# MAGPIE-ICL/synthPy

Measured on AMD Instinct MI355X. Metric: ray-steps/sec (+ rays/sec to detector), 1e7 rays x 512^3 volume, higher is better.
Workload: dtype f64

## Files before the change

include/synthray.h:

```cpp
#ifndef SYNTHRAY_H
#define SYNTHRAY_H

#include <stddef.h>
#include <stdint.h>

#ifdef __cplusplus
extern "C" {
#endif

#define SR_OK 0
#define SR_ERR_INVALID (-1)
#define SR_ERR_HIP (-2)
#define SR_ERR_RCCL (-3)
#define SR_ERR_STATE (-4)

typedef struct sr_volume sr_volume;
typedef struct sr_rays sr_rays;
typedef struct sr_image sr_image;
typedef struct sr_comm sr_comm;

int sr_init(int device);
int sr_device_count(void);
int sr_synchronize(void);
int sr_device_memory(int64_t *free_bytes, int64_t *total_bytes);
// ... 85 lines not shown
} sr_trace_stats;

int sr_trace(const sr_volume *v, const double *s0, int64_t n_rays, const sr_trace_params *p,
             double *sf, double *rf, double *Jf, sr_trace_stats *stats);

int sr_ray_to_jones(const double *sf, int64_t n_rays, double extent, int probing_axis, int row_order,
                    double *rf, double *Jf);

int sr_rays_create(sr_rays **out, int64_t n_rays);
int sr_rays_upload(sr_rays *r, const double *s0);
int sr_rays_upload_part(sr_rays *r, const double *s0, int64_t n, int64_t first, int last);
int sr_rays_generate(sr_rays *r, int beam_type, double size_a, double size_b, double divergence, double ne_extent,
                     int probing_axis, uint64_t seed, uint64_t first_ray);
int sr_rays_trace(sr_rays *r, const sr_volume *v, const sr_trace_params *p, sr_trace_stats *stats);
int sr_rays_trace_stats(sr_rays *r, sr_trace_stats *stats);

int sr_rays_tile_segments(const sr_rays *r);
int sr_rays_tile_records(const sr_rays *r);
double sr_tile_min_density(void);
int sr_rays_download(const sr_rays *r, double *sf, double *rf, double *Jf);
int sr_rays_download_s0(const sr_rays *r, double *s0);
int sr_rays_error_bound(const sr_rays *r, float *bound);
int64_t sr_rays_count(const sr_rays *r);
int sr_rays_handoff_download(const sr_rays *r, double *rec);
int sr_rays_set_bbox(sr_rays *r, const double *bbox);
int sr_rays_get_bbox(const sr_rays *r, double *bbox, int *known);
int sr_rays_handoff_upload(sr_rays *r, const double *rec);
int sr_rays_handoff_send(sr_rays *r, sr_comm *comm, int peer);
int sr_rays_handoff_recv(sr_rays *r, sr_comm *comm, int peer);
void sr_rays_destroy(sr_rays *r);

enum {
  SR_OP_DIST = 0,
  SR_OP_LENS = 1,
  SR_OP_CIRC_AP = 2,
  SR_OP_CIRC_STOP = 3,
  SR_OP_RECT_AP = 4,
  SR_OP_KNIFE = 5,
  SR_OP_SCALE = 6,
  SR_OP_PHASE = 7
};
typedef struct {
  int32_t op;
  int32_t iarg;
  double a;
  double b;
// ... 72 lines not shown
```

synthpy_amd/_ffi.py:

```python
from __future__ import annotations

import ctypes as C
import os

import numpy as np

_HERE = os.path.dirname(os.path.abspath(__file__))
LIB_PATH = os.environ.get("SYNTHRAY_LIB") or os.path.join(_HERE, "libsynthray.so")


class SynthrayError(RuntimeError):
    """A libsynthray call returned a negative status."""


class Optic(C.Structure):
    _fields_ = [("op", C.c_int32), ("iarg", C.c_int32), ("a", C.c_double), ("b", C.c_double)]


class TraceParams(C.Structure):
    _fields_ = [("t_end", C.c_double), ("extent", C.c_double), ("dt", C.c_double), ("probing_axis", C.c_int32),
                ("row_order", C.c_int32), ("substeps", C.c_int32), ("sort_rays", C.c_int32), ("precision", C.c_int32),
                ("handoff", C.c_int32)]


# ... 57 lines not shown
    "sr_volume_sample_aux": (_i, [_vp, _vp, _i64, _vp]),
    "sr_volume_project": (_i, [_vp, _vp, C.POINTER(C.c_uint32)]),
    "sr_volume_omega": (_d, [_vp]),
    "sr_volume_bytes": (_i64, [_vp]),
    "sr_volume_destroy": (None, [_vp]),
    "sr_trace": (_i, [_vp, _vp, _i64, C.POINTER(TraceParams), _vp, _vp, _vp, C.POINTER(TraceStats)]),
    "sr_ray_to_jones": (_i, [_vp, _i64, _d, _i, _i, _vp, _vp]),
    "sr_rays_create": (_i, [_pp, _i64]),
    "sr_rays_download_s0": (_i, [_vp, _vp]),
    "sr_rays_error_bound": (_i, [_vp, _vp]),
    "sr_rays_generate": (_i, [_vp, _i, _d, _d, _d, _d, _i, C.c_uint64, C.c_uint64]),
    "sr_rays_upload": (_i, [_vp, _vp]),
    "sr_rays_upload_part": (_i, [_vp, _vp, _i64, _i64, _i]),
    "sr_rays_trace": (_i, [_vp, _vp, C.POINTER(TraceParams), C.POINTER(TraceStats)]),
    "sr_release_caches": (_i, []),
    "sr_rays_trace_stats": (_i, [_vp, C.POINTER(TraceStats)]),
    "sr_rays_tile_segments": (_i, [_vp]),
    "sr_tile_min_density": (_d, []),
    "sr_rays_tile_records": (_i, [_vp]),
    "sr_rays_set_bbox": (_i, [_vp, _vp]),
    "sr_rays_get_bbox": (_i, [_vp, _vp, C.POINTER(C.c_int)]),
    "sr_rays_download": (_i, [_vp, _vp, _vp, _vp]),
    "sr_rays_count": (_i64, [_vp]),
    "sr_rays_destroy": (None, [_vp]),
    "sr_optics": (_i, [C.POINTER(Optic), _i, _d, _i64, _vp, _vp, _vp, _vp]),
    "sr_hist2d": (_i, [_vp, _vp, _i64, _i, _i, _d, _d, _d, _d, _vp]),
    "sr_interferogram": (_i, [_vp, _vp, _vp, _i64, _i, _i, _d, _d, _d, _d, _vp, _vp]),
    "sr_interfere_ref_beam": (_i, [_vp, _vp, _i64, _d, _d, _vp]),
    "sr_image_create": (_i, [_pp, _i, _i, _i, _d, _d, _d, _d]),
    "sr_image_zero": (_i, [_vp]),
    "sr_image_download": (_i, [_vp, _vp]),
    "sr_image_amplitude": (_i, [_vp, _vp]),
    "sr_image_counts_f64": (_i, [_vp, _vp]),
    "sr_rays_optics": (_i, [_vp, C.POINTER(Optic), _i, C.POINTER(DepositParams), _vp, _vp]),
    "sr_image_bytes": (_i64, [_vp]),
    "sr_image_destroy": (None, [_vp]),
    "sr_rays_deposit": (_i, [_vp, C.POINTER(Optic), _i, C.POINTER(DepositParams), _vp, C.POINTER(DepositStats)]),
    "sr_rays_refine": (_i, [_vp, _i, _vp, _vp, _vp, C.POINTER(C.c_int64)]),
    "sr_image_create_intensity": (_i, [_pp, _i, _i, _i, _d, _d, _d, _d]),
    "sr_rays_deposit_intensity": (_i, [_vp, C.POINTER(Optic), _i, _vp, _i, _i, _vp, C.POINTER(DepositStats)]),
    "sr_intensity2d": (_i, [_vp, _vp, _vp, _i64, _vp, _i, _i, _i, _d, _d, _d, _d, _vp]),
    "sr_image_rotation": (_i, [_vp, _i, _i, _d, _vp]),
    "sr_comm_unique_id": (_i, [_vp]),
    "sr_comm_create": (_i, [_pp, _vp, _i, _i]),
    "sr_image_reduce": (_i, [_vp, _vp, _i]),
    "sr_comm_ranks": (_i, [_vp, C.POINTER(C.c_int), C.POINTER(C.c_int)]),
# ... 45 lines not shown
```

synthpy_amd/csrc/common.hpp:

```cpp
#pragma once
#include <hip/hip_runtime.h>

#include <cstdarg>
#include <cstdint>
#include <cstdio>
#include <map>
#include <string>
#include <type_traits>
#include <vector>

#include "synthray.h"

namespace sr {

constexpr double kC = 299792458.0;

void set_error(const char *fmt, ...);
int fail(int code, const char *fmt, ...);

#define SR_HIP(call)                                                                         \
  do {                                                                                       \
    hipError_t e_ = (call);                                                                  \
    if (e_ != hipSuccess)                                                                    \
      return sr::fail(SR_ERR_HIP, "%s failed: %s (%s:%d)", #call, hipGetErrorString(e_),     \
// ... 99 lines not shown
  mutable std::map<int, void *> step_tabs;
};

struct sr_rays {
  int64_t n = 0;
  int64_t cap = 0;
  double bbox[6] = {0, 0, 0, 0, 0, 0};
  bool have_bbox = false;
  bool bbox_given = false;
  double *s0 = nullptr;
  double *sf = nullptr;
  double *rf = nullptr;
  double *Jf = nullptr;
  uint32_t *perm = nullptr;
  uint32_t *keys = nullptr;
  uint32_t *bins = nullptr;
  uint32_t *sort_tmp = nullptr;
  int64_t bins_cap = 0;
  uint32_t *fb_list = nullptr;
  unsigned long long *counters = nullptr;
  double *rec = nullptr;
  double *rec2 = nullptr;
  uint32_t *order2 = nullptr;
  double *strag_rec = nullptr;
  unsigned long long *strag_snap = nullptr;
  int strag_snap_cap = 0;
  bool have_s0 = false, traced = false, sorted = false, have_rec = false;
  bool counters_carry = false;
  int tile_segs = 0;
  int tile_segs_run = 0;
  bool tile_rec = false;
  float *guard = nullptr;
  const sr_volume *last_vol = nullptr;
  sr_trace_params last_p{};
  void *guard_set = nullptr;
  std::vector<char> guard_set_host;
  bool guard_live = false;
  double guard_len = 0;
};

namespace sr {
int retrace_f64(const sr_rays *r, const uint32_t *list, const unsigned long long *count);
int download_rows(const sr_rays *r, double *sf, double *rf, double *Jf, int64_t ld, int64_t off, double *staging);
}

struct sr_image {
// ... 8 lines not shown
```

synthpy_amd/csrc/trace.hip:

```cpp
#include <algorithm>
#include <cmath>
#include <cstdlib>
#include <cstring>

#include "common.hpp"

namespace {

struct VolDev {
  const float4 *P;
  const float *L;
  const double *g[3];
  const double *rg[3];
  int na, nb, nc;
  double omega;
  const double *K;
  const double *Q;
  double verdet;
  int64_t OS;
  const double *R;
};

constexpr int64_t kSC = 8;
__device__ __forceinline__ int64_t col8(const VolDev &V, int ib, int ic) { return ((int64_t)ib * V.nc + ic) * 8; }
// ... 236 lines not shown
    run += v[q];
  }
  const int lane = threadIdx.x & 63, wid = threadIdx.x >> 6;
  uint32_t incl = run;
  for (int off = 1; off < 64; off <<= 1) {
    const uint32_t up = __shfl_up(incl, off, 64);
    if (lane >= off) incl += up;
  }
  if (lane == 63) wsum[wid] = incl;
  __syncthreads();
  uint32_t woff = 0;
  for (int w = 0; w < wid; ++w) woff += wsum[w];
  uint32_t ex = woff + incl - run;
#pragma unroll
  for (int q = 0; q < 8; ++q) {
    if (base + q < n) bins[base + q] = ex;
    ex += v[q];
  }
  if (threadIdx.x == 255) sums[blockIdx.x] = woff + incl;
}
__global__ void k_scan_add(uint32_t *__restrict__ bins, int64_t n, const uint32_t *__restrict__ sums) {
  const int64_t i = blockIdx.x * (int64_t)blockDim.x + threadIdx.x;
  if (i < n) bins[i] += sums[i / kScanPerBlock];
}

__device__ __forceinline__ void project(int a, int row_order, double extent, int64_t N, int64_t j, double pa, double pb,
                                        double pc, double va, double vb, double vc, double amp, double phase, double pol,
                                        double *__restrict__ rf, double *__restrict__ Jf) {
  const double tb = (pa - extent) / va;
  double q0 = pb - vb * tb, q2 = pc - vc * tb;
  double a1 = atan(vb / va), a3 = atan(vc / va);
  if (a == 1 && row_order == SR_ROWS_LEGACY) {
    double t = q0;
    q0 = q2;
    q2 = t;
    t = a1;
    a1 = a3;
    a3 = t;
  }
  rf[j] = q0;
  rf[N + j] = a1;
  rf[2 * N + j] = q2;
  rf[3 * N + j] = a3;
  if (Jf) {
    double sp, cp, so, co;
    sincos(phase, &sp, &cp);
// ... 385 lines not shown
    sr::dev_free(r->bins);
    r->bins = nullptr;
    r->bins_cap = 0;
    int rc = sr::dev_alloc(&r->bins, (size_t)(ncount + nsb));
    if (rc) return rc;
    r->bins_cap = ncount + nsb;
  }
  if (!r->sort_tmp) {
    int rc = sr::dev_alloc(&r->sort_tmp, (size_t)2 * (size_t)std::max(r->cap, N));
    if (rc) return rc;
  }
  uint32_t *sums = r->bins + ncount, *tkeys = r->sort_tmp, *trays = r->sort_tmp + N;
  hipLaunchKernelGGL(k_bin_count, dim3(n_wg), dim3(256), 0, st, (const uint32_t *)r->keys, N, lo_bits, n_coarse, r->bins, n_wg);
  hipLaunchKernelGGL(k_scan_blocks, dim3((unsigned)nsb), dim3(256), 0, st, r->bins, ncount, sums);
  hipLaunchKernelGGL(k_scan, dim3(1), dim3(1024), 0, st, sums, nsb);
  hipLaunchKernelGGL(k_scan_add, dim3(sr::grid_for(ncount, 256)), dim3(256), 0, st, r->bins, ncount, (const uint32_t *)sums);
  hipLaunchKernelGGL(k_bin_coarse, dim3(n_wg), dim3(256), 0, st, (const uint32_t *)r->keys, N, lo_bits, n_coarse,
                     (const uint32_t *)r->bins, n_wg, tkeys, trays);
  hipLaunchKernelGGL(k_bin_fine, dim3((unsigned)n_coarse), dim3(1024), 0, st, (const uint32_t *)tkeys, (const uint32_t *)trays, N,
                     lo_bits, n_coarse, (const uint32_t *)r->bins, n_wg, out);
  return SR_OK;
}

int bin_by_band(sr_rays *r, const sr_volume *v, const TileGeom &g, const double *rec, uint32_t *out, hipStream_t st) {
  const int64_t N = r->n;
  const int64_t n_bands = (v->nb - 1 + g.band - 1) / g.band;
  const int64_t n_keys = n_bands * (int64_t)(v->nc - 1) * g.band;
  int bits = 1;
  while (((int64_t)1 << bits) < n_keys) ++bits;
  const int shift = std::max(0, bits - 22);
  const int64_t key_max = ((n_keys - 1) >> shift) + 1;
  bits = 1;
  while (((int64_t)1 << bits) <= key_max) ++bits;
  const int lo_bits = std::min(11, (bits + 1) / 2);
  const int n_coarse = (int)(key_max >> lo_bits) + 1;
  SR_CHECK(n_coarse <= kBinMaxDigits + 1, "band key of %lld does not fit the LDS counters of the ray binning", (long long)key_max);
  const unsigned nblk = sr::grid_for(N, 256);
  if (rec)
    hipLaunchKernelGGL(k_keys_band_rec, dim3(nblk), dim3(256), 0, st, vol_dev(v), rec, N, g.band, (uint32_t)key_max, shift, r->keys);
  else
    hipLaunchKernelGGL(k_keys_band, dim3(nblk), dim3(256), 0, st, vol_dev(v), (const double *)r->s0, N, v->axis, g.band, (uint32_t)key_max,
                       shift, r->keys);
  return bin_rays(r, N, lo_bits, n_coarse, out, st);
}

constexpr double kTileMinDensity = 8.0;
struct TilePlan {
  TileGeom g;
  int seg;
  bool rec;
};

struct TraceKnobs {
  int f64_tile = -1;
  bool tile_records = true;
  bool strag_beside = true;
  bool aux_one_pass = false;
  TileGeom tile{};
  int tile_seg = 0;
  std::vector<double> cuts;
};
TraceKnobs trace_knobs() {
  TraceKnobs k;
  if (const char *e = getenv("SYNTHRAY_F64_TILE")) k.f64_tile = e[0] == '0' ? 0 : (e[0] == '1' ? 1 : -1);
  if (const char *e = getenv("SYNTHRAY_TILE_RECORDS")) k.tile_records = e[0] != '0';
  if (const char *e = getenv("SYNTHRAY_STRAGGLERS")) k.strag_beside = e[0] != 's';
  if (const char *e = getenv("SYNTHRAY_AUX_ONE_PASS")) k.aux_one_pass = e[0] == '1';
  if (const char *e = getenv("SYNTHRAY_TILE")) {
    int a, b, c, d, f;
    if (sscanf(e, "%d,%d,%d,%d,%d", &a, &b, &c, &d, &f) == 5 && a >= 2 && b >= 2 && c >= 0 && d >= 1 && f >= 1 && a * b <= SR_TILE_THREADS) {
      k.tile = TileGeom{a, b, c, d};
      k.tile_seg = f;
    }
  }
  if (const char *e = getenv("SYNTHRAY_TILE_CUTS"))
    for (const char *q = e; *q;) {
      char *end = nullptr;
      const double x = strtod(q, &end);
      if (end == q) break;
      k.cuts.push_back(x);
      q = *end == ',' ? end + 1 : end;
    }
  return k;
}
double beam_cells(const sr_rays *r, const sr_volume *v) {
  const double all = (double)(v->nb - 1) * (double)(v->nc - 1);
  if (!r || !r->have_bbox) return all;
  double cells = 1.0;
  for (int q = 1; q <= 2; ++q) {
    const int phys = (v->axis + q) % 3, n = q == 1 ? v->nb : v->nc;
// ... 79 lines not shown

void launch_planes64(const sr_volume *v, const sr_trace_params *p, const TraceKnobs &knobs, const TraceArgs &A, hipStream_t st);

std::vector<double> tile_cut_weights(int n_seg) {
  std::vector<double> w((size_t)n_seg, 1.0);
  for (int q = 0; q < n_seg; ++q) w[(size_t)q] = n_seg > 1 ? 1.3 - 0.6 * q / (n_seg - 1) : 1.0;
  return w;
}

std::vector<int> tile_cuts(int steps, int n_seg, const TraceKnobs &knobs) {
  bool given = (int)knobs.cuts.size() == n_seg;
  for (double x : knobs.cuts) given = given && x > 0;
  const std::vector<double> w = given ? knobs.cuts : tile_cut_weights(n_seg);
  std::vector<int> cut((size_t)n_seg + 1, 0);
  double tot = 0, acc = 0;
  for (double x : w) tot += x;
  for (int q = 0; q < n_seg; ++q) {
    acc += w[(size_t)q];
    cut[(size_t)q + 1] = q + 1 == n_seg ? steps : std::min(steps - (n_seg - 1 - q), std::max(cut[(size_t)q] + 1, (int)std::lround(steps * acc / tot)));
  }
  return cut;
}

int tile_buffers(sr_rays *r, size_t cap, int n_seg, bool second) {
  int rc = SR_OK;
  if (!r->rec && (rc = sr::dev_alloc(&r->rec, 10 * cap))) return rc;
  if (second) {
    if (!r->rec2 && (rc = sr::dev_alloc(&r->rec2, 10 * cap))) return rc;
    if (!r->order2 && (rc = sr::dev_alloc(&r->order2, cap))) return rc;
  }
  if (!r->strag_rec && (rc = sr::dev_alloc(&r->strag_rec, 10 * cap))) return rc;
  if (r->strag_snap_cap < n_seg + 1) {
    sr::dev_free(r->strag_snap);
    r->strag_snap_cap = 0;
    if ((rc = sr::dev_alloc(&r->strag_snap, (size_t)std::max(n_seg + 1, 64)))) return rc;
    r->strag_snap_cap = std::max(n_seg + 1, 64);
  }
  return SR_OK;
}

int launch_tile(const TileArgs &T, bool phase, bool aux, bool rec, size_t lds, hipStream_t st) {
  const unsigned grid = ((T.A.n_blocks + 7) / 8) * 8;
  hipError_t err = hipSuccess;
  with_flags(
      [&](auto ph, auto ax, auto rc) {
        if constexpr (!(ax.value && rc.value)) {
          auto *kernel = &k_trace_tile<ph.value, ax.value, rc.value>;
          static const hipError_t whole_lds =
// ... 27 lines not shown
  F.A = A;
  F.A.rec = r->rec;
  F.A.guard = r->guard;
  F.strag = r->strag_rec;
  F.cap = (int64_t)cap;
  F.exit_rec = ho_exit ? 1 : 0;
  F.slab = slab ? 1 : 0;
  hipLaunchKernelGGL(k_strag_finish, dim3(sr::grid_for(A.N, 256)), dim3(256), 0, st, F);
}

int trace_tiled(sr_rays *r, const sr_volume *v, const sr_trace_params *p, const TraceKnobs &knobs, const TilePlan &tp, TraceArgs &A,
                hipStream_t st) {
  const int64_t N = r->n;
  sr::Context &c = sr::ctx();
  hipStream_t side = c.side[c.current];
  hipEvent_t ev_go = c.side_ev[c.current][0], ev_done = c.side_ev[c.current][1];
  const int steps = v->na - 1;
  const int n_seg = (steps + tp.seg - 1) / tp.seg;
  const bool phase = v->L != nullptr, aux = v->K != nullptr || v->Q != nullptr;
  const size_t lds = tile_lds_bytes(tp.g, (steps + n_seg - 1) / n_seg + 1, aux, tp.rec);
  const bool ho_enter = (p->handoff & SR_HANDOFF_ENTER) != 0, ho_exit = (p->handoff & SR_HANDOFF_EXIT) != 0;
  const bool slab = v->is_slab || p->handoff;
  const size_t cap = (size_t)std::max(r->cap, N);
  int rc = tile_buffers(r, cap, n_seg, n_seg > 1 || ho_enter);
  if (rc) return rc;
  unsigned long long *strag_count = r->counters + 8;
  SR_HIP(hipMemsetAsync(strag_count, 0, sizeof(unsigned long long), st));
  SR_HIP(hipMemsetAsync(r->strag_snap, 0, sizeof(unsigned long long), st));
  const std::vector<int> cut = tile_cuts(steps, n_seg, knobs);
  const bool timed = n_seg <= sr::kMaxTileSegs;
  TileArgs T{};
  T.G = tp.g;
  T.exit_rec = ho_exit ? 1 : 0;
  T.slab = slab ? 1 : 0;
  T.A = A;
  T.A.guard = r->guard;
  T.A.n_blocks = sr::grid_for(N, SR_TILE_THREADS);
  T.perm_out = r->perm;
  T.strag_rec = r->strag_rec;
  T.strag_cap = (int64_t)cap;
  T.strag_count = strag_count;
  for (int q = 0; q < n_seg; ++q) {
    T.k0 = cut[(size_t)q];
    T.k1 = cut[(size_t)q + 1];
    T.first = q == 0 && !ho_enter;
    T.last = q + 1 == n_seg;
    if (T.first) {
      T.rec_in = nullptr;
      T.order = nullptr;
      T.A.rec = r->rec;
    } else {
      rc = bin_by_band(r, v, tp.g, r->rec, r->order2, st);
      if (rc) return rc;
      T.rec_in = r->rec;
      T.order = r->order2;
      T.A.rec = r->rec2;
    }
    if (timed) SR_HIP(hipEventRecord(c.ev[4 + 2 * q], st));
    if ((rc = launch_tile(T, phase, aux, tp.rec, lds, st))) return rc;
    if (timed) SR_HIP(hipEventRecord(c.ev[5 + 2 * q], st));
    hipLaunchKernelGGL(k_strag_snap, dim3(1), dim3(1), 0, st, (const unsigned long long *)strag_count, r->strag_snap, q, r->counters + 3);
    hipStream_t ss = st;
    if (knobs.strag_beside) {
      SR_HIP(hipEventRecord(ev_go, st));
      SR_HIP(hipStreamWaitEvent(side, ev_go, 0));
      ss = side;
    }
    launch_planes64(v, p, knobs, straggler_args(A, r, cap, q, T.k0, ho_exit), ss);
    if (!T.first) std::swap(r->rec, r->rec2);
  }
  if (knobs.strag_beside) {
    SR_HIP(hipEventRecord(ev_done, side));
    SR_HIP(hipStreamWaitEvent(st, ev_done, 0));
  }
  launch_strag_finish(A, r, cap, ho_exit, slab, st);
  A.guard = r->guard;
  r->tile_segs = timed ? n_seg : 0;
  r->tile_segs_run = n_seg;
  r->tile_rec = tp.rec;
  return SR_OK;
}

int make_trace_args(const sr_rays *r, const sr_volume *v, const sr_trace_params *p, TraceArgs &A) {
  const int64_t N = r->n;
// ... 212 lines not shown
  sr_trace_params p = r->last_p;
  p.precision = SR_PREC_F64;
  hipStream_t st = sr::ctx().stream;
  TraceArgs A;
  int rc = make_trace_args(r, v, &p, A);
  if (rc) return rc;
  A.step_stripe = 2;
  A.in_list = list;
  A.in_count = count;
  A.out_list = r->keys;
  A.out_count = r->counters + 5;
  launch_planes64(v, &p, knobs, A, st);
  launch_time(v, A, st);
  SR_HIP(hipGetLastError());
  return SR_OK;
}

extern "C" {

void sr_rays_destroy(sr_rays *r) {
  if (!r) return;
  for (void *q : {(void *)r->s0, (void *)r->sf, (void *)r->rf, (void *)r->Jf, (void *)r->perm, (void *)r->keys, (void *)r->bins,
                  (void *)r->sort_tmp, (void *)r->fb_list, (void *)r->counters, (void *)r->rec, (void *)r->rec2, (void *)r->order2,
                  (void *)r->strag_rec, (void *)r->strag_snap, (void *)r->guard, r->guard_set})
    sr::dev_free(q);
  delete r;
}

int sr_rays_create(sr_rays **out, int64_t n) {
  SR_CHECK(out != nullptr, "sr_rays_create: NULL out");
  *out = nullptr;
  SR_CHECK(n >= 0 && n < (int64_t)0xFFFFFFFFll, "sr_rays_create: ray count %lld out of range", (long long)n);
  int rc = sr::ensure_init();
  if (rc) return rc;
  sr_rays *r = new sr_rays();
  r->n = n;
  r->cap = n;
  const size_t m = (size_t)(n > 0 ? n : 1);
  if ((rc = sr::dev_alloc(&r->s0, 9 * m)) || (rc = sr::dev_alloc(&r->sf, 9 * m)) || (rc = sr::dev_alloc(&r->rf, 4 * m)) ||
      (rc = sr::dev_alloc(&r->Jf, 4 * m)) || (rc = sr::dev_alloc(&r->perm, m)) || (rc = sr::dev_alloc(&r->keys, m)) ||
      (rc = sr::dev_alloc(&r->fb_list, m)) || (rc = sr::dev_alloc(&r->counters, sr::kCounterWords)) ||
      (rc = sr::dev_alloc(&r->guard, m))) {
    sr_rays_destroy(r);
    return rc;
  }
  *out = r;
  return SR_OK;
}

int64_t sr_rays_count(const sr_rays *r) { return r ? r->n : 0; }

int sr_rays_upload(sr_rays *r, const double *s0) {
  SR_CHECK(r && s0, "sr_rays_upload: NULL argument");
  r->have_bbox = r->bbox_given = false;
  if (r->n > 0) {
    hipStream_t st = sr::ctx().stream;
    int rc = sr::upload_sync(r->s0, s0, sizeof(double) * 9 * (size_t)r->n, st);
    if (!rc) rc = read_bbox(r, st);
    if (rc) return rc;
  }
  r->have_s0 = true;
  r->traced = false;
  return SR_OK;
}

int sr_rays_upload_part(sr_rays *r, const double *s0, int64_t n, int64_t first, int last) {
  SR_CHECK(r && (s0 || n == 0), "sr_rays_upload_part: NULL argument");
  SR_CHECK(n >= 0 && first >= 0 && first + n <= r->n, "sr_rays_upload_part: rays %lld .. %lld of a bundle of %lld", (long long)first,
           (long long)(first + n), (long long)r->n);
  hipStream_t st = sr::ctx().stream;
  r->have_bbox = r->bbox_given = false;
  r->have_s0 = false;
  r->traced = false;
  if (n > 0) {
// ... 41 lines not shown
  r->tile_rec = false;
  TilePlan tplan;
  bool tiled = tile_plan(r, v, p, N, knobs, true, tplan);
  if (tiled && tplan.rec) {
    bool have = false;
    int rc = tile_records(v, knobs, st, have);
    if (rc) return rc;
    if (!have) tiled = tile_plan(r, v, p, N, knobs, false, tplan);
  }

  SR_HIP(hipEventRecord(c.ev[0], st));
  if (r->counters_carry)
    SR_HIP(hipMemsetAsync(r->counters + 1, 0, 2 * sizeof(unsigned long long), st));
  else
    SR_HIP(hipMemsetAsync(r->counters, 0, sr::kCounterWords * sizeof(unsigned long long), st));
  if (p->handoff && !r->rec) {
    int rc = sr::dev_alloc(&r->rec, (size_t)10 * (size_t)std::max(r->cap, N));
    if (rc) return rc;
  }
  if (ho_enter && tiled) {
  } else if (ho_enter) {
    hipLaunchKernelGGL(k_perm_from_rec, dim3(nblk), dim3(block), 0, st, (const double *)r->rec, N, r->perm);
  } else if (p->sort_rays && tiled) {
    int rc = bin_by_band(r, v, tplan.g, nullptr, r->perm, st);
    if (rc) return rc;
  } else if (p->sort_rays) {
    int bits = 1;
    while ((1 << bits) < std::max(v->nb - 1, v->nc - 1)) ++bits;
    const int shift = std::max(0, bits - 11);
    bits -= shift;
    const uint32_t oob_key = (uint32_t)1 << (2 * bits);
    hipLaunchKernelGGL(k_keys, dim3(nblk), dim3(block), 0, st, V, (const double *)r->s0, N, v->axis, oob_key, shift, r->keys);
    int rc = bin_rays(r, N, bits, (1 << bits) + 1, r->perm, st);
    if (rc) return rc;
  } else {
    hipLaunchKernelGGL(k_iota, dim3(nblk), dim3(block), 0, st, r->perm, N);
  }

  TraceArgs A;
  {
    int rc = make_trace_args(r, v, p, A);
    if (rc) return rc;
  }
  SR_HIP(hipEventRecord(c.ev[1], st));
  const bool aux = v->K != nullptr || v->Q != nullptr;
  const bool mixed = p->precision == SR_PREC_MIXED && !aux && p->substeps == 1;
  if (mixed) {
// ... 182 lines not shown
```

synthpy_amd/csrc/trace_tile.inc:

```
struct TileGeom {
  int tb, tc;
  int halo;
  int band;
};

struct TileArgs {
  TraceArgs A;
  TileGeom G;
  int k0, k1;
  int first, last;
  int exit_rec, slab;
  int rot;
  unsigned block0;
  const double *rec_in;
  const uint32_t *order;
  uint32_t *perm_out;
  double *strag_rec;
  int64_t strag_cap;
  unsigned long long *strag_count;
};

constexpr int kRecColD = (1024 + 80) / 8;
__host__ __device__ constexpr int tile_rec(bool aux, bool rec = false) { return aux ? 38 : (rec ? 16 : 18); }

__host__ __device__ inline size_t tile_lds_bytes(const TileGeom &g, int seg_steps, bool aux = false, bool rec = false) {
  const size_t tables = (size_t)(2 * (g.tb + 1) + 2 * (g.tc + 1) + 4);
  (void)seg_steps;
  const size_t head = rec ? (((tables * sizeof(double)) + 1023) & ~(size_t)1023) / sizeof(double) : ((tables + 1) & ~(size_t)1);
  if (rec) return sizeof(double) * (head + (size_t)5 * g.tc * kRecColD);
  return sizeof(double) * (head + (size_t)5 * g.tb * g.tc * tile_rec(aux, rec));
}

__device__ __forceinline__ uint32_t band_key(int ib, int ic, int ncc, int band) {
  const int bnd = ib / band, row = ib - bnd * band;
  const int col = (bnd & 1) ? ncc - 1 - ic : ic;
  return ((uint32_t)bnd * (uint32_t)ncc + (uint32_t)col) * (uint32_t)band + (uint32_t)row;
}

__global__ void k_keys_band(VolDev V, const double *__restrict__ s0, int64_t N, int axis, int band, uint32_t oob_key, int shift,
                            uint32_t *__restrict__ keys) {
  const int64_t i = blockIdx.x * (int64_t)blockDim.x + threadIdx.x;
  if (i >= N) return;
  const int b = (axis + 1) % 3, c = (axis + 2) % 3;
  double pa = s0[axis * N + i], pb = s0[b * N + i], pc = s0[c * N + i];
  const double va = s0[(3 + axis) * N + i], vb = s0[(3 + b) * N + i], vc = s0[(3 + c) * N + i];
  const double ga0 = V.g[0][0];
  if (va > 0 && pa < ga0) {
    const double tau = (ga0 - pa) / va;
    pb = pb + vb * tau;
    pc = pc + vc * tau;
  }
  const double gb0 = V.g[1][0], gbL = V.g[1][V.nb - 1], gc0 = V.g[2][0], gcL = V.g[2][V.nc - 1];
  uint32_t key = oob_key;
  if (pb >= gb0 && pb <= gbL && pc >= gc0 && pc <= gcL) {
    const int ib = find_cell(V.g[1], V.nb, pb, gb0, (V.nb - 1) / (gbL - gb0));
    const int ic = find_cell(V.g[2], V.nc, pc, gc0, (V.nc - 1) / (gcL - gc0));
    key = band_key(ib, ic, V.nc - 1, band) >> shift;
  }
  keys[i] = key;
}

__global__ void k_keys_band_rec(VolDev V, const double *__restrict__ rec, int64_t N, int band, uint32_t oob_key, int shift,
                                uint32_t *__restrict__ keys) {
  const int64_t j = blockIdx.x * (int64_t)blockDim.x + threadIdx.x;
  if (j >= N) return;
  const double pb = rec[j], pc = rec[N + j], va = rec[2 * N + j];
  const double gb0 = V.g[1][0], gbL = V.g[1][V.nb - 1], gc0 = V.g[2][0], gcL = V.g[2][V.nc - 1];
  uint32_t key = oob_key;
  if (va > 0 && pb >= gb0 && pb <= gbL && pc >= gc0 && pc <= gcL) {
    const int ib = find_cell(V.g[1], V.nb, pb, gb0, (V.nb - 1) / (gbL - gb0));
    const int ic = find_cell(V.g[2], V.nc, pc, gc0, (V.nc - 1) / (gcL - gc0));
    key = band_key(ib, ic, V.nc - 1, band) >> shift;
  }
  keys[j] = key;
}

__global__ void k_strag_snap(const unsigned long long *count, unsigned long long *snap, int q, unsigned long long *total) {
  const unsigned long long c = *count;
  snap[q + 1] = c;
  *total += c - snap[q];
}

struct StragFinish {
  TraceArgs A;
  const double *strag;
  int64_t cap;
  int exit_rec, slab;
};
__global__ __launch_bounds__(256) void k_strag_finish(StragFinish F) {
  const TraceArgs &A = F.A;
  const int64_t N = A.N;
  const int64_t j = blockIdx.x * (int64_t)blockDim.x + threadIdx.x;
  const bool gone = j < N && A.rec[2 * N + j] == -__builtin_inf();
  double y[9];
#pragma unroll
  for (int row = 0; row < 9; ++row) y[row] = __builtin_nan("");
  if (gone) {
// ... 716 lines not shown
    }
    const bool finished = alive && y6 <= B.t_end;
    if (finished) {
      double amp = y7, pol = y8;
      if (!AUX) {
        if (tail_args->first) {
          amp = B.s0[6 * N + i];
          pol = B.s0[8 * N + i];
        } else {
          amp = B.rec[7 * N + j];
          pol = B.rec[8 * N + j];
        }
      }
      const double rem = B.t_end - y6;
      write_outputs(B, j, fma(y2, rem, B.V.g[0][B.V.na - 1]), fma(y3, rem, y0), fma(y4, rem, y1), y2, y3, y4, y5, amp, pol);
      tot = (unsigned long long)(B.V.na - 1);
    }
    if (tail_args->slab) {
      if (have && !finished && !lost && !gone) write_lost(B, j);
    } else {
      queue_push(B.out_count, B.out_list, have && !finished && !lost && !gone, (uint32_t)j);
    }
  }
  for (int off = 32; off > 0; off >>= 1) tot += __shfl_down(tot, off, 64);
  if ((threadIdx.x & 63) == 0 && tot) atomicAdd(sr::stripe(B.counters, B.step_stripe), tot);
}
```

synthpy_amd/engine.py:

```python
from __future__ import annotations

import ctypes as C
import os
import weakref
from dataclasses import dataclass

import numpy as np

from . import _ffi
from ._ffi import check, f32, f64, lib, ptr

c = 299792458.0

OP_DIST, OP_LENS, OP_CIRC_AP, OP_CIRC_STOP, OP_RECT_AP, OP_KNIFE, OP_SCALE, OP_PHASE = range(8)
ROWS_LEGACY, ROWS_JAX = 0, 1
IMG_COUNTS, IMG_COMPLEX, IMG_INTENSITY = 0, 1, 2
VOL_PHASE = 1

_AXES = {"x": 0, "y": 1, "z": 2}


def axis_index(probing_direction) -> int:
    if isinstance(probing_direction, str) and probing_direction in _AXES:
        return _AXES[probing_direction]
# ... 357 lines not shown

class RayBundle:

    def __init__(self, n_rays: int):
        self.n = int(n_rays)
        self._h = C.c_void_p()
        self._volume, self.retraced = None, 0
        self.generation = 0
        self.holders = weakref.WeakSet()
        check(lib.sr_rays_create(C.byref(self._h), self.n))

    @property
    def alive(self) -> bool:
        return bool(getattr(self, "_h", None))

    def upload(self, s0):
        s0 = f64(s0)
        if s0.shape != (9, self.n):
            raise ValueError(f"s0 must have shape (9, {self.n}), got {s0.shape}")
        self.generation += 1
        check(lib.sr_rays_upload(self._h, ptr(s0)))
        return self

    def upload_part(self, s0, first, last=False):
        s0 = f64(s0)
        if s0.ndim != 2 or s0.shape[0] != 9 or first < 0 or first + s0.shape[1] > self.n:
            raise ValueError(f"part of shape {s0.shape} at ray {first} does not fit a bundle of {self.n} rays")
        self.generation += 1
        check(lib.sr_rays_upload_part(self._h, ptr(s0), int(s0.shape[1]), int(first), 1 if last else 0))
        return self

    def generate(self, beam_size, divergence, ne_extent, beam_type="circular", probing_direction="z", seed=0, first_ray=0,
                 radial_law="legacy"):
        if beam_type == "circular":
            if radial_law not in ("legacy", "power"):
                raise ValueError("radial_law must be 'legacy' or 'power'")
            kind, a, b = (0 if radial_law == "legacy" else 3), float(beam_size), 0.0
        elif beam_type == "linear":
            kind, a, b = 2, float(beam_size), 0.0
        elif beam_type == "square":
            kind, a, b = 1, float(beam_size), float(beam_size)
        elif beam_type == "rectangular":
            kind, a, b = 1, float(beam_size[0]), float(beam_size[1])
        else:
            raise ValueError(f"beam_type {beam_type!r}: 'circular', 'square', 'rectangular' or 'linear' on the device")
        self.generation += 1
# ... 313 lines not shown
```

Measured before the change: 118.0 billion.

## Fuse per-segment ray re-binning into tile tail via wave-aggregated counting sort

Between tiled trace segments, rays were re-sorted by band key with a separate key kernel followed by a multi-pass radix binning. Now the tile kernel's tail computes each surviving ray's next band key and its rank inside that key using wave-aggregated atomics. A single scan kernel, which also takes over the straggler snapshot, and a single place kernel then build the next order directly. This is meant to cut kernel launches and global passes over the keys, at the cost of atomic contention on hot cells, an extra cell-count buffer, and a key count bounded by LDS. It also adds a resize API and an opt-in fused first binning.

```diff
diff --git a/include/synthray.h b/include/synthray.h
--- a/include/synthray.h
+++ b/include/synthray.h
@@ -131,6 +131,7 @@
 int sr_rays_download_s0(const sr_rays *r, double *s0);
 int sr_rays_error_bound(const sr_rays *r, float *bound);
 int64_t sr_rays_count(const sr_rays *r);
+int sr_rays_resize(sr_rays *r, int64_t n);
 int sr_rays_handoff_download(const sr_rays *r, double *rec);
 int sr_rays_set_bbox(sr_rays *r, const double *bbox);
 int sr_rays_get_bbox(const sr_rays *r, double *bbox, int *known);
diff --git a/synthpy_amd/_ffi.py b/synthpy_amd/_ffi.py
--- a/synthpy_amd/_ffi.py
+++ b/synthpy_amd/_ffi.py
@@ -103,6 +103,7 @@
     "sr_rays_get_bbox": (_i, [_vp, _vp, C.POINTER(C.c_int)]),
     "sr_rays_download": (_i, [_vp, _vp, _vp, _vp]),
     "sr_rays_count": (_i64, [_vp]),
+    "sr_rays_resize": (_i, [_vp, _i64]),
     "sr_rays_destroy": (None, [_vp]),
     "sr_optics": (_i, [C.POINTER(Optic), _i, _d, _i64, _vp, _vp, _vp, _vp]),
     "sr_hist2d": (_i, [_vp, _vp, _i64, _i, _i, _d, _d, _d, _d, _vp]),
diff --git a/synthpy_amd/csrc/common.hpp b/synthpy_amd/csrc/common.hpp
--- a/synthpy_amd/csrc/common.hpp
+++ b/synthpy_amd/csrc/common.hpp
@@ -145,6 +145,8 @@
   double *rec = nullptr;
   double *rec2 = nullptr;
   uint32_t *order2 = nullptr;
+  uint32_t *cells = nullptr;
+  int64_t cells_cap = 0;
   double *strag_rec = nullptr;
   unsigned long long *strag_snap = nullptr;
   int strag_snap_cap = 0;
diff --git a/synthpy_amd/csrc/trace.hip b/synthpy_amd/csrc/trace.hip
--- a/synthpy_amd/csrc/trace.hip
+++ b/synthpy_amd/csrc/trace.hip
@@ -282,6 +282,81 @@
 __global__ void k_scan_add(uint32_t *__restrict__ bins, int64_t n, const uint32_t *__restrict__ sums) {
   const int64_t i = blockIdx.x * (int64_t)blockDim.x + threadIdx.x;
   if (i < n) bins[i] += sums[i / kScanPerBlock];
+}
+
+constexpr int kRebinMaxSums = (1 << 22) / kScanPerBlock + 1;
+constexpr int kPlacePerLane = 8;
+__global__ __launch_bounds__(256) void k_rebin_scan(uint32_t *__restrict__ counts, int64_t n, uint32_t *__restrict__ starts,
+                                                    uint32_t *__restrict__ sums, const unsigned long long *strag_count,
+                                                    unsigned long long *snap, int q, unsigned long long *total) {
+  __shared__ uint32_t wsum[4];
+  if (strag_count && blockIdx.x == 0 && threadIdx.x == 0) {
+    const unsigned long long c = *strag_count;
+    snap[q + 1] = c;
+    *total += c - snap[q];
+  }
+  const int64_t base = (int64_t)blockIdx.x * kScanPerBlock + (int64_t)threadIdx.x * 8;
+  uint32_t v[8], run = 0;
+#pragma unroll
+  for (int e = 0; e < 8; ++e) {
+    v[e] = base + e < n ? counts[base + e] : 0u;
+    run += v[e];
+  }
+  const int lane = threadIdx.x & 63, wid = threadIdx.x >> 6;
+  uint32_t incl = run;
+  for (int off = 1; off < 64; off <<= 1) {
+    const uint32_t up = __shfl_up(incl, off, 64);
+    if (lane >= off) incl += up;
+  }
+  if (lane == 63) wsum[wid] = incl;
+  __syncthreads();
+  uint32_t woff = 0;
+  for (int w = 0; w < wid; ++w) woff += wsum[w];
+  uint32_t ex = woff + incl - run;
+#pragma unroll
+  for (int e = 0; e < 8; ++e) {
+    if (base + e < n) {
+      starts[base + e] = ex;
+      counts[base + e] = 0u;
+    }
+    ex += v[e];
+  }
+  if (threadIdx.x == 255) sums[blockIdx.x] = woff + incl;
+}
+__global__ __launch_bounds__(256) void k_rebin_place(const uint32_t *__restrict__ keys, const uint32_t *__restrict__ ranks, int64_t N,
+                                                     const uint32_t *__restrict__ starts, const uint32_t *__restrict__ sums, int n_sums,
+                                                     uint32_t *__restrict__ order) {
+  __shared__ uint32_t first[kRebinMaxSums];
+  __shared__ uint32_t wsum[4];
+  const int per = (n_sums + 255) / 256, t0 = (int)threadIdx.x * per;
+  uint32_t run = 0;
+  for (int e = 0; e < per; ++e) run += t0 + e < n_sums ? sums[t0 + e] : 0u;
+  const int lane = threadIdx.x & 63, wid = threadIdx.x >> 6;
+  uint32_t incl = run;
+  for (int off = 1; off < 64; off <<= 1) {
+    const uint32_t up = __shfl_up(incl, off, 64);
+    if (lane >= off) incl += up;
+  }
+  if (lane == 63) wsum[wid] = incl;
+  __syncthreads();
+  uint32_t ex = incl - run;
+  for (int w = 0; w < wid; ++w) ex += wsum[w];
+  for (int e = 0; e < per; ++e)
+    if (t0 + e < n_sums) {
+      first[t0 + e] = ex;
+      ex += sums[t0 + e];
+    }
+  __syncthreads();
+  const int64_t base = (int64_t)blockIdx.x * (256 * kPlacePerLane) + threadIdx.x;
+#pragma unroll
+  for (int e = 0; e < kPlacePerLane; ++e) {
+    const int64_t j = base + e * 256;
+    if (j < N) {
+      const uint32_t key = keys[j];
+      const uint32_t pos = first[key / kScanPerBlock] + starts[key] + ranks[j];
+      if (pos < (uint32_t)N) order[pos] = (uint32_t)j;
+    }
+  }
 }
 
 __device__ __forceinline__ void project(int a, int row_order, double extent, int64_t N, int64_t j, double pa, double pb,
@@ -713,26 +788,83 @@
   return SR_OK;
 }
 
-int bin_by_band(sr_rays *r, const sr_volume *v, const TileGeom &g, const double *rec, uint32_t *out, hipStream_t st) {
-  const int64_t N = r->n;
+struct BandKeys {
+  int shift = 0;
+  int64_t key_max = 0;
+  int lo_bits = 0, n_coarse = 0;
+};
+BandKeys band_keys(const sr_volume *v, const TileGeom &g) {
+  BandKeys k;
   const int64_t n_bands = (v->nb - 1 + g.band - 1) / g.band;
   const int64_t n_keys = n_bands * (int64_t)(v->nc - 1) * g.band;
   int bits = 1;
   while (((int64_t)1 << bits) < n_keys) ++bits;
-  const int shift = std::max(0, bits - 22);
-  const int64_t key_max = ((n_keys - 1) >> shift) + 1;
+  k.shift = std::max(0, bits - 22);
+  k.key_max = ((n_keys - 1) >> k.shift) + 1;
   bits = 1;
-  while (((int64_t)1 << bits) <= key_max) ++bits;
-  const int lo_bits = std::min(11, (bits + 1) / 2);
-  const int n_coarse = (int)(key_max >> lo_bits) + 1;
-  SR_CHECK(n_coarse <= kBinMaxDigits + 1, "band key of %lld does not fit the LDS counters of the ray binning", (long long)key_max);
+  while (((int64_t)1 << bits) <= k.key_max) ++bits;
+  k.lo_bits = std::min(11, (bits + 1) / 2);
+  k.n_coarse = (int)(k.key_max >> k.lo_bits) + 1;
+  return k;
+}
+
+struct RebinPlan {
+  int64_t n_cells = 0, n_sums = 0;
+  explicit RebinPlan(const BandKeys &k) : n_cells(k.key_max + 1), n_sums((k.key_max + 1 + kScanPerBlock - 1) / kScanPerBlock) {}
+  int64_t words() const { return 2 * n_cells + n_sums; }
+  uint32_t *counts(const sr_rays *r) const { return r->cells; }
+  uint32_t *starts(const sr_rays *r) const { return r->cells + n_cells; }
+  uint32_t *sums(const sr_rays *r) const { return r->cells + 2 * n_cells; }
+};
+int rebin_buffers(sr_rays *r, size_t cap, const RebinPlan &rp) {
+  int rc = SR_OK;
+  SR_CHECK(rp.n_sums <= kRebinMaxSums, "%lld band keys do not fit the re-binning's scan", (long long)rp.n_cells);
+  if (!r->sort_tmp && (rc = sr::dev_alloc(&r->sort_tmp, 2 * cap))) return rc;
+  if (r->cells_cap < rp.words()) {
+    sr::dev_free(r->cells);
+    r->cells = nullptr;
+    r->cells_cap = 0;
+    if ((rc = sr::dev_alloc(&r->cells, (size_t)rp.words()))) return rc;
+    r->cells_cap = rp.words();
+  }
+  return SR_OK;
+}
+void launch_rebin_scan(const sr_rays *r, const RebinPlan &rp, const unsigned long long *strag_count, int q, hipStream_t st) {
+  hipLaunchKernelGGL(k_rebin_scan, dim3((unsigned)rp.n_sums), dim3(256), 0, st, rp.counts(r), rp.n_cells, rp.starts(r), rp.sums(r), strag_count,
+                     r->strag_snap, q, r->counters + 3);
+}
+void launch_rebin_place(const sr_rays *r, const RebinPlan &rp, int64_t N, uint32_t *out, hipStream_t st) {
+  hipLaunchKernelGGL(k_rebin_place, dim3(sr::grid_for(N, 256 * kPlacePerLane)), dim3(256), 0, st, (const uint32_t *)r->keys,
+                     (const uint32_t *)r->sort_tmp, N, (const uint32_t *)rp.starts(r), (const uint32_t *)rp.sums(r), (int)rp.n_sums, out);
+}
+
+int bin_by_band(sr_rays *r, const sr_volume *v, const TileGeom &g, const double *rec, uint32_t *out, bool fused, hipStream_t st) {
+  const int64_t N = r->n;
+  const BandKeys k = band_keys(v, g);
+  if (fused) {
+    const RebinPlan rp(k);
+    int rc = rebin_buffers(r, (size_t)std::max(r->cap, N), rp);
+    if (rc) return rc;
+    SR_HIP(hipMemsetAsync(rp.counts(r), 0, sizeof(uint32_t) * (size_t)rp.n_cells, st));
+    const unsigned grid = sr::grid_for(N, 256);
+    if (rec)
+      hipLaunchKernelGGL(k_keys_rank_band<true>, dim3(grid), dim3(256), 0, st, vol_dev(v), rec, N, v->axis, g.band, (uint32_t)k.key_max, k.shift,
+                         r->keys, r->sort_tmp, rp.counts(r));
+    else
+      hipLaunchKernelGGL(k_keys_rank_band<false>, dim3(grid), dim3(256), 0, st, vol_dev(v), (const double *)r->s0, N, v->axis, g.band,
+                         (uint32_t)k.key_max, k.shift, r->keys, r->sort_tmp, rp.counts(r));
+    launch_rebin_scan(r, rp, nullptr, 0, st);
+    launch_rebin_place(r, rp, N, out, st);
+    return SR_OK;
+  }
+  SR_CHECK(k.n_coarse <= kBinMaxDigits + 1, "band key of %lld does not fit the LDS counters of the ray binning", (long long)k.key_max);
   const unsigned nblk = sr::grid_for(N, 256);
   if (rec)
-    hipLaunchKernelGGL(k_keys_band_rec, dim3(nblk), dim3(256), 0, st, vol_dev(v), rec, N, g.band, (uint32_t)key_max, shift, r->keys);
+    hipLaunchKernelGGL(k_keys_band_rec, dim3(nblk), dim3(256), 0, st, vol_dev(v), rec, N, g.band, (uint32_t)k.key_max, k.shift, r->keys);
   else
-    hipLaunchKernelGGL(k_keys_band, dim3(nblk), dim3(256), 0, st, vol_dev(v), (const double *)r->s0, N, v->axis, g.band, (uint32_t)key_max,
-                       shift, r->keys);
-  return bin_rays(r, N, lo_bits, n_coarse, out, st);
+    hipLaunchKernelGGL(k_keys_band, dim3(nblk), dim3(256), 0, st, vol_dev(v), (const double *)r->s0, N, v->axis, g.band, (uint32_t)k.key_max,
+                       k.shift, r->keys);
+  return bin_rays(r, N, k.lo_bits, k.n_coarse, out, st);
 }
 
 constexpr double kTileMinDensity = 8.0;
@@ -747,6 +879,8 @@
   bool tile_records = true;
   bool strag_beside = true;
   bool aux_one_pass = false;
+  bool rebin_fused = true;
+  bool first_fused = false;
   TileGeom tile{};
   int tile_seg = 0;
   std::vector<double> cuts;
@@ -757,6 +891,8 @@
   if (const char *e = getenv("SYNTHRAY_TILE_RECORDS")) k.tile_records = e[0] != '0';
   if (const char *e = getenv("SYNTHRAY_STRAGGLERS")) k.strag_beside = e[0] != 's';
   if (const char *e = getenv("SYNTHRAY_AUX_ONE_PASS")) k.aux_one_pass = e[0] == '1';
+  if (const char *e = getenv("SYNTHRAY_TILE_REBIN")) k.rebin_fused = e[0] != 's';
+  if (const char *e = getenv("SYNTHRAY_TILE_FIRST_BIN")) k.first_fused = e[0] == 'f';
   if (const char *e = getenv("SYNTHRAY_TILE")) {
     int a, b, c, d, f;
     if (sscanf(e, "%d,%d,%d,%d,%d", &a, &b, &c, &d, &f) == 5 && a >= 2 && b >= 2 && c >= 0 && d >= 1 && f >= 1 && a * b <= SR_TILE_THREADS) {
@@ -882,8 +1018,9 @@
   return cut;
 }
 
-int tile_buffers(sr_rays *r, size_t cap, int n_seg, bool second) {
+int tile_buffers(sr_rays *r, size_t cap, int n_seg, bool second, const RebinPlan *rebin) {
   int rc = SR_OK;
+  if (rebin && (rc = rebin_buffers(r, cap, *rebin))) return rc;
   if (!r->rec && (rc = sr::dev_alloc(&r->rec, 10 * cap))) return rc;
   if (second) {
     if (!r->rec2 && (rc = sr::dev_alloc(&r->rec2, 10 * cap))) return rc;
@@ -957,8 +1094,12 @@
   const bool ho_enter = (p->handoff & SR_HANDOFF_ENTER) != 0, ho_exit = (p->handoff & SR_HANDOFF_EXIT) != 0;
   const bool slab = v->is_slab || p->handoff;
   const size_t cap = (size_t)std::max(r->cap, N);
-  int rc = tile_buffers(r, cap, n_seg, n_seg > 1 || ho_enter);
+  const bool fused = knobs.rebin_fused && n_seg > 1;
+  const BandKeys bk = band_keys(v, tp.g);
+  const RebinPlan rp(bk);
+  int rc = tile_buffers(r, cap, n_seg, n_seg > 1 || ho_enter, fused ? &rp : nullptr);
   if (rc) return rc;
+  if (fused) SR_HIP(hipMemsetAsync(rp.counts(r), 0, sizeof(uint32_t) * (size_t)rp.n_cells, st));
   unsigned long long *strag_count = r->counters + 8;
   SR_HIP(hipMemsetAsync(strag_count, 0, sizeof(unsigned long long), st));
   SR_HIP(hipMemsetAsync(r->strag_snap, 0, sizeof(unsigned long long), st));
@@ -975,6 +1116,10 @@
   T.strag_rec = r->strag_rec;
   T.strag_cap = (int64_t)cap;
   T.strag_count = strag_count;
+  T.ranks = r->sort_tmp;
+  T.cell_count = rp.counts(r);
+  T.oob_key = (uint32_t)bk.key_max;
+  T.key_shift = bk.shift;
   for (int q = 0; q < n_seg; ++q) {
     T.k0 = cut[(size_t)q];
     T.k1 = cut[(size_t)q + 1];
@@ -985,16 +1130,24 @@
       T.order = nullptr;
       T.A.rec = r->rec;
     } else {
-      rc = bin_by_band(r, v, tp.g, r->rec, r->order2, st);
-      if (rc) return rc;
+      if (fused && q > 0) {
+        launch_rebin_place(r, rp, N, r->order2, st);
+      } else {
+        rc = bin_by_band(r, v, tp.g, r->rec, r->order2, knobs.first_fused, st);
+        if (rc) return rc;
+      }
       T.rec_in = r->rec;
       T.order = r->order2;
       T.A.rec = r->rec2;
     }
+    T.keys = fused && !T.last ? r->keys : nullptr;
     if (timed) SR_HIP(hipEventRecord(c.ev[4 + 2 * q], st));
     if ((rc = launch_tile(T, phase, aux, tp.rec, lds, st))) return rc;
     if (timed) SR_HIP(hipEventRecord(c.ev[5 + 2 * q], st));
-    hipLaunchKernelGGL(k_strag_snap, dim3(1), dim3(1), 0, st, (const unsigned long long *)strag_count, r->strag_snap, q, r->counters + 3);
+    if (T.keys)
+      launch_rebin_scan(r, rp, strag_count, q, st);
+    else
+      hipLaunchKernelGGL(k_strag_snap, dim3(1), dim3(1), 0, st, (const unsigned long long *)strag_count, r->strag_snap, q, r->counters + 3);
     hipStream_t ss = st;
     if (knobs.strag_beside) {
       SR_HIP(hipEventRecord(ev_go, st));
@@ -1253,7 +1406,7 @@
   if (!r) return;
   for (void *q : {(void *)r->s0, (void *)r->sf, (void *)r->rf, (void *)r->Jf, (void *)r->perm, (void *)r->keys, (void *)r->bins,
                   (void *)r->sort_tmp, (void *)r->fb_list, (void *)r->counters, (void *)r->rec, (void *)r->rec2, (void *)r->order2,
-                  (void *)r->strag_rec, (void *)r->strag_snap, (void *)r->guard, r->guard_set})
+                  (void *)r->strag_rec, (void *)r->strag_snap, (void *)r->cells, (void *)r->guard, r->guard_set})
     sr::dev_free(q);
   delete r;
 }
@@ -1281,6 +1434,16 @@
 
 int64_t sr_rays_count(const sr_rays *r) { return r ? r->n : 0; }
 
+int sr_rays_resize(sr_rays *r, int64_t n) {
+  SR_CHECK(r != nullptr, "sr_rays_resize: NULL bundle");
+  SR_CHECK(n >= 0 && n <= r->cap, "sr_rays_resize: %lld rays in a bundle made for %lld", (long long)n, (long long)r->cap);
+  r->n = n;
+  r->have_s0 = r->have_rec = r->traced = r->sorted = false;
+  r->have_bbox = r->bbox_given = false;
+  r->guard_live = false;
+  return SR_OK;
+}
+
 int sr_rays_upload(sr_rays *r, const double *s0) {
   SR_CHECK(r && s0, "sr_rays_upload: NULL argument");
   r->have_bbox = r->bbox_given = false;
@@ -1368,7 +1531,7 @@
   } else if (ho_enter) {
     hipLaunchKernelGGL(k_perm_from_rec, dim3(nblk), dim3(block), 0, st, (const double *)r->rec, N, r->perm);
   } else if (p->sort_rays && tiled) {
-    int rc = bin_by_band(r, v, tplan.g, nullptr, r->perm, st);
+    int rc = bin_by_band(r, v, tplan.g, nullptr, r->perm, knobs.first_fused, st);
     if (rc) return rc;
   } else if (p->sort_rays) {
     int bits = 1;
diff --git a/synthpy_amd/csrc/trace_tile.inc b/synthpy_amd/csrc/trace_tile.inc
--- a/synthpy_amd/csrc/trace_tile.inc
+++ b/synthpy_amd/csrc/trace_tile.inc
@@ -18,6 +18,9 @@
   double *strag_rec;
   int64_t strag_cap;
   unsigned long long *strag_count;
+  uint32_t *keys, *ranks, *cell_count;
+  uint32_t oob_key;
+  int key_shift;
 };
 
 constexpr int kRecColD = (1024 + 80) / 8;
@@ -37,10 +40,30 @@
   return ((uint32_t)bnd * (uint32_t)ncc + (uint32_t)col) * (uint32_t)band + (uint32_t)row;
 }
 
-__global__ void k_keys_band(VolDev V, const double *__restrict__ s0, int64_t N, int axis, int band, uint32_t oob_key, int shift,
-                            uint32_t *__restrict__ keys) {
-  const int64_t i = blockIdx.x * (int64_t)blockDim.x + threadIdx.x;
-  if (i >= N) return;
+__device__ __forceinline__ uint32_t wave_key_rank(bool have, uint32_t key, uint32_t *counts) {
+  const int lane = threadIdx.x & 63;
+  unsigned long long todo = __ballot(have);
+  int lead = 0;
+  uint32_t place = 0, size = 0;
+  while (todo != 0ull) {
+    const int l = __ffsll((long long)todo) - 1;
+    const uint32_t k = (uint32_t)__builtin_amdgcn_readlane((int)key, l);
+    const bool mine = have && key == k;
+    const unsigned long long m = __ballot(mine);
+    if (mine) {
+      lead = l;
+      place = (uint32_t)__popcll(m & ((1ull << lane) - 1ull));
+      size = (uint32_t)__popcll(m);
+    }
+    todo &= ~m;
+  }
+  uint32_t base = 0;
+  if (have && lane == lead) base = atomicAdd(counts + key, size);
+  return __shfl(base, lead, 64) + place;
+}
+
+__device__ __forceinline__ uint32_t entry_band_key(const VolDev &V, const double *__restrict__ s0, int64_t N, int64_t i, int axis, int band,
+                                                   uint32_t oob_key, int shift) {
   const int b = (axis + 1) % 3, c = (axis + 2) % 3;
   double pa = s0[axis * N + i], pb = s0[b * N + i], pc = s0[c * N + i];
   const double va = s0[(3 + axis) * N + i], vb = s0[(3 + b) * N + i], vc = s0[(3 + c) * N + i];
@@ -57,14 +80,17 @@
     const int ic = find_cell(V.g[2], V.nc, pc, gc0, (V.nc - 1) / (gcL - gc0));
     key = band_key(ib, ic, V.nc - 1, band) >> shift;
   }
-  keys[i] = key;
-}
-
-__global__ void k_keys_band_rec(VolDev V, const double *__restrict__ rec, int64_t N, int band, uint32_t oob_key, int shift,
-                                uint32_t *__restrict__ keys) {
-  const int64_t j = blockIdx.x * (int64_t)blockDim.x + threadIdx.x;
-  if (j >= N) return;
-  const double pb = rec[j], pc = rec[N + j], va = rec[2 * N + j];
+  return key;
+}
+
+__global__ void k_keys_band(VolDev V, const double *__restrict__ s0, int64_t N, int axis, int band, uint32_t oob_key, int shift,
+                            uint32_t *__restrict__ keys) {
+  const int64_t i = blockIdx.x * (int64_t)blockDim.x + threadIdx.x;
+  if (i >= N) return;
+  keys[i] = entry_band_key(V, s0, N, i, axis, band, oob_key, shift);
+}
+
+__device__ __forceinline__ uint32_t record_band_key(const VolDev &V, double pb, double pc, double va, int band, uint32_t oob_key, int shift) {
   const double gb0 = V.g[1][0], gbL = V.g[1][V.nb - 1], gc0 = V.g[2][0], gcL = V.g[2][V.nc - 1];
   uint32_t key = oob_key;
   if (va > 0 && pb >= gb0 && pb <= gbL && pc >= gc0 && pc <= gcL) {
@@ -72,7 +98,27 @@
     const int ic = find_cell(V.g[2], V.nc, pc, gc0, (V.nc - 1) / (gcL - gc0));
     key = band_key(ib, ic, V.nc - 1, band) >> shift;
   }
-  keys[j] = key;
+  return key;
+}
+__global__ void k_keys_band_rec(VolDev V, const double *__restrict__ rec, int64_t N, int band, uint32_t oob_key, int shift,
+                                uint32_t *__restrict__ keys) {
+  const int64_t j = blockIdx.x * (int64_t)blockDim.x + threadIdx.x;
+  if (j >= N) return;
+  keys[j] = record_band_key(V, rec[j], rec[N + j], rec[2 * N + j], band, oob_key, shift);
+}
+template <bool REC>
+__global__ __launch_bounds__(256) void k_keys_rank_band(VolDev V, const double *__restrict__ src, int64_t N, int axis, int band, uint32_t oob_key,
+                                                         int shift, uint32_t *__restrict__ keys, uint32_t *__restrict__ ranks,
+                                                         uint32_t *__restrict__ counts) {
+  const int64_t j = blockIdx.x * (int64_t)blockDim.x + threadIdx.x;
+  const bool have = j < N;
+  uint32_t key = oob_key;
+  if (have) key = REC ? record_band_key(V, src[j], src[N + j], src[2 * N + j], band, oob_key, shift) : entry_band_key(V, src, N, j, axis, band, oob_key, shift);
+  const uint32_t rank = wave_key_rank(have, key, counts);
+  if (have) {
+    keys[j] = key;
+    ranks[j] = rank;
+  }
 }
 
 __global__ void k_strag_snap(const unsigned long long *count, unsigned long long *snap, int q, unsigned long long *total) {
@@ -835,6 +881,15 @@
       queue_push(B.out_count, B.out_list, have && !finished && !lost && !gone, (uint32_t)j);
     }
   }
+  if (tail_args->keys) {
+    uint32_t key = tail_args->oob_key;
+    if (have && !lost && (alive || gone)) key = record_band_key(B.V, y0, y1, y2, tail_args->G.band, tail_args->oob_key, tail_args->key_shift);
+    const uint32_t rank = wave_key_rank(have, key, tail_args->cell_count);
+    if (have) {
+      tail_args->keys[j] = key;
+      tail_args->ranks[j] = rank;
+    }
+  }
   for (int off = 32; off > 0; off >>= 1) tot += __shfl_down(tot, off, 64);
   if ((threadIdx.x & 63) == 0 && tot) atomicAdd(sr::stripe(B.counters, B.step_stripe), tot);
 }
diff --git a/synthpy_amd/engine.py b/synthpy_amd/engine.py
--- a/synthpy_amd/engine.py
+++ b/synthpy_amd/engine.py
@@ -403,6 +403,12 @@
         check(lib.sr_rays_upload(self._h, ptr(s0)))
         return self
 
+    def resize(self, n_rays: int):
+        self.generation += 1
+        check(lib.sr_rays_resize(self._h, int(n_rays)))
+        self.n = int(n_rays)
+        return self
+
     def upload_part(self, s0, first, last=False):
         s0 = f64(s0)
         if s0.ndim != 2 or s0.shape[0] != 9 or first < 0 or first + s0.shape[1] > self.n:
```

Result: slower. 116.8 billion (-1.0%).
